# will-assistant/open-speech

Measured on AMD Instinct MI355X. Metric: audio-sec/sec (whisper-large-v3-turbo, 30 s clips, greedy), higher is better.
Workload: dtype f16; 1 GPU; large-v3-turbo: 64 x 30 s clips per GPU per step, mel+encoder+greedy decode (max_length 448); clips_per_gpu=64, global_batch=64, parallelism=dp1, lanes_per_gpu=3

## Files before the change

### include/osw.h

```cpp
#ifndef OSW_H
#define OSW_H

#include <stdint.h>

#ifdef __cplusplus
extern "C" {
#endif

#define OSW_OK 0
#define OSW_EINVAL (-22)
#define OSW_ENOMEM (-12)
#define OSW_EHIP (-100)
#define OSW_ESTATE (-101)
#define OSW_ECAPTURE (-102)

typedef struct osw_ctx osw_ctx;

typedef struct osw_dims {
    int32_t n_mels, n_audio_ctx, n_audio_state, n_audio_head, n_audio_layer;
    int32_t n_vocab, n_text_ctx, n_text_state, n_text_head, n_text_layer;
} osw_dims;

typedef struct osw_window {
    int32_t clip;
// ... 200 lines not shown

#define OSW_EPI_F16 0
#define OSW_EPI_F16_GELU 1
#define OSW_EPI_F32_RESID 2
#define OSW_EPI_F32_GELU_POS 3
#define OSW_EPI_F32 4
#define OSW_EPI_HEADS 5
typedef struct osw_enc_gemm_desc {
    int32_t M, N, K, variant, epi;
    int32_t heads_T, heads_H, heads_nb;
    int64_t lda, a_grp_rows, a_grp_stride;
    int64_t a_count;
    int64_t ldc, c_grp_rows, c_grp_stride, c_offset;
    int64_t c_bytes;
    int64_t pos_count;
    const void* A;
    const void* W;
    const float* bias;
    const float* pos;
    const int32_t* heads_slot;
    void* C;
} osw_enc_gemm_desc;
int osw_debug_enc_gemm(osw_ctx* ctx, const osw_enc_gemm_desc* desc);
int osw_debug_enc_layernorm(osw_ctx* ctx, int32_t M, int32_t M_alloc, int32_t D, const float* x, const float* gain,
                            const float* shift, void* y);

int osw_debug_get_logmel(osw_ctx* ctx, int32_t clip, float* out, int64_t out_floats, float* clip_max);
int osw_debug_mel_windows(osw_ctx* ctx, const osw_window* windows, int32_t n, void* out_halfs, int64_t out_count);

int osw_debug_hold_capture(osw_ctx* ctx, int32_t hold_ms);

int osw_set_profiling(osw_ctx* ctx, int32_t enable);
int osw_get_profile(osw_ctx* ctx, osw_profile* out);
void* osw_stream(osw_ctx* ctx);

int osw_ingest_mean_square(int32_t device, const int16_t* pcm, int64_t n_frames, int32_t channels, float* out_mean);
int osw_ingest_apply_gain(int32_t device, const int16_t* pcm, int64_t n_frames, int32_t channels, int32_t apply_gain,
                          float gain, int16_t* out);
int osw_ingest_resample(int32_t device, const int16_t* pcm, int64_t n_in, int32_t up, int32_t down, const float* h,
                        int32_t n_h, int16_t* out, int64_t n_out);

#ifdef __cplusplus
}
#endif
#endif
```

### open-speech_amd/_lib.py

```python
from __future__ import annotations

import ctypes as C
import os
import threading

_HERE = os.path.dirname(os.path.abspath(__file__))
LIB_PATH = os.environ.get("OSW_LIB", os.path.join(_HERE, "lib", "libosw_hip.so"))

OSW_OK = 0


class osw_dims(C.Structure):
    _fields_ = [(n, C.c_int32) for n in ("n_mels", "n_audio_ctx", "n_audio_state", "n_audio_head", "n_audio_layer",
                                          "n_vocab", "n_text_ctx", "n_text_state", "n_text_head", "n_text_layer")]


class osw_window(C.Structure):
    _fields_ = [("clip", C.c_int32), ("seek", C.c_int32), ("segment_size", C.c_int32)]


class osw_decode_opts(C.Structure):
    _fields_ = [("task_token", C.c_int32), ("language_token", C.c_int32), ("suppress_blank", C.c_int32),
                ("without_timestamps", C.c_int32), ("max_initial_timestamp_index", C.c_int32),
                ("max_length", C.c_int32), ("suppress_tokens", C.POINTER(C.c_int32)), ("n_suppress", C.c_int32),
# ... 118 lines not shown
                                      C.c_int32, C.c_int32, C.c_int32, P(C.c_float)]),
    "osw_debug_dec_xattn_windows": (C.c_int, [C.c_void_p, P(C.c_float), C.c_int32, P(C.c_float), C.c_void_p,
                                              C.c_void_p, C.c_int32, P(C.c_int32), C.c_int32, C.c_int32, C.c_int32,
                                              P(C.c_float)]),
    "osw_debug_dec_self_attn": (C.c_int, [C.c_void_p, P(C.c_float), C.c_int32, P(C.c_float), C.c_void_p, C.c_void_p,
                                          C.c_int32, P(C.c_int32), C.c_int32, P(C.c_int32), C.c_int32,
                                          P(C.c_float)]),
    "osw_debug_dec_gemm": (C.c_int, [C.c_void_p, C.c_int32, C.c_int32, C.c_int32, C.c_int32, C.c_void_p, C.c_void_p,
                                     C.c_void_p, C.c_int32, P(C.c_float), C.c_int64, P(C.c_int32)]),
    "osw_debug_dec_gemm_quant": (C.c_int, [C.c_void_p, C.c_int32, C.c_int32, C.c_int32, C.c_int32, C.c_void_p,
                                        C.c_void_p, C.c_void_p, P(C.c_float), C.c_int32, P(C.c_float), C.c_int64,
                                        P(C.c_int32)]),
    "osw_debug_dec_gemm_time": (C.c_int, [C.c_void_p, C.c_int32, C.c_int32, C.c_int32, C.c_void_p, C.c_void_p,
                                          C.c_void_p, P(C.c_float), C.c_int32, C.c_int32, C.c_int32, P(C.c_float),
                                          P(C.c_float)]),
    "osw_debug_logits_profile": (C.c_int, [C.c_void_p, P(C.c_double), P(C.c_int64)]),
    "osw_debug_dec_resln": (C.c_int, [C.c_void_p, C.c_int32, C.c_int32, C.c_int32, C.c_int32, P(C.c_float), C.c_int32,
                                      P(C.c_float), P(C.c_float), P(C.c_float), P(C.c_float), C.c_void_p,
                                      P(C.c_float), P(C.c_int32), P(C.c_int32), C.c_int32, C.c_int32, C.c_int32,
                                      C.c_void_p, C.c_int32, C.c_int32, P(C.c_float), C.c_void_p, C.c_void_p,
                                      P(C.c_float), C.c_int64, P(C.c_int32)]),
    "osw_debug_dec_gelu": (C.c_int, [C.c_void_p, C.c_int32, C.c_int32, C.c_int32, P(C.c_float), C.c_int32,
                                     P(C.c_float), C.c_void_p, C.c_int32, C.c_int32, C.c_void_p, C.c_void_p,
                                     P(C.c_float), C.c_int64, P(C.c_int32)]),
    "osw_debug_enc_gemm": (C.c_int, [C.c_void_p, P(osw_enc_gemm_desc)]),
    "osw_debug_enc_layernorm": (C.c_int, [C.c_void_p, C.c_int32, C.c_int32, C.c_int32, P(C.c_float), P(C.c_float),
                                          P(C.c_float), C.c_void_p]),
    "osw_debug_get_logmel": (C.c_int, [C.c_void_p, C.c_int32, P(C.c_float), C.c_int64, P(C.c_float)]),
    "osw_debug_mel_windows": (C.c_int, [C.c_void_p, P(osw_window), C.c_int32, C.c_void_p, C.c_int64]),
    "osw_debug_hold_capture": (C.c_int, [C.c_void_p, C.c_int32]),
    "osw_set_encoder_baton_min": (C.c_int, [C.c_void_p, C.c_int32]),
    "osw_set_profiling": (C.c_int, [C.c_void_p, C.c_int32]),
    "osw_get_profile": (C.c_int, [C.c_void_p, P(osw_profile)]),
    "osw_stream": (C.c_void_p, [C.c_void_p]),
    "osw_ingest_mean_square": (C.c_int, [C.c_int32, P(C.c_int16), C.c_int64, C.c_int32, P(C.c_float)]),
    "osw_ingest_apply_gain": (C.c_int, [C.c_int32, P(C.c_int16), C.c_int64, C.c_int32, C.c_int32, C.c_float,
                                        P(C.c_int16)]),
    "osw_ingest_resample": (C.c_int, [C.c_int32, P(C.c_int16), C.c_int64, C.c_int32, C.c_int32, P(C.c_float),
                                      C.c_int32, P(C.c_int16), C.c_int64]),
}
EXPORTED = tuple(_SIGS)

_lib = None
_lock = threading.Lock()


def load() -> C.CDLL:
    global _lib
    with _lock:
        if _lib is not None:
            return _lib
        if not os.path.exists(LIB_PATH):
            raise RuntimeError(f"libosw_hip.so not found at {LIB_PATH}: build it with `python __graft_entry__.py` "
                               "or `make -C open-speech_amd/csrc` (there is no CPU fallback)")
        lib = C.CDLL(LIB_PATH)
        for name, (res, args) in _SIGS.items():
            fn = getattr(lib, name)
            fn.restype = res
            fn.argtypes = args
        _lib = lib
        return lib


OSW_EINVAL = -22
OSW_EHIP = -100
OSW_ESTATE = -101
# ... 25 lines not shown
```

### open-speech_amd/csrc/common.h

```cpp
#pragma once
#include <hip/hip_runtime.h>
#include <hip/hip_fp16.h>
#include <stdint.h>

namespace osw {

typedef _Float16 h16;
typedef _Float16 h16x8 __attribute__((ext_vector_type(8)));
typedef _Float16 h16x4 __attribute__((ext_vector_type(4)));
typedef _Float16 h16x2 __attribute__((ext_vector_type(2)));
typedef float f32x4 __attribute__((ext_vector_type(4)));
typedef float f32x2 __attribute__((ext_vector_type(2)));
typedef float f32x16 __attribute__((ext_vector_type(16)));
typedef short s16x4 __attribute__((vector_size(8)));

#define OSW_LDS __attribute__((address_space(3)))

__device__ __forceinline__ int float_to_ordered(float f) {
    int i = __float_as_int(f);
    return i >= 0 ? i : (i ^ 0x7fffffff);
}
__device__ __forceinline__ float ordered_to_float(int i) {
    return __int_as_float(i >= 0 ? i : (i ^ 0x7fffffff));
}
// ... 64 lines not shown
    EPI_F32_GELU_POS = 3,
    EPI_F32 = 4,
    EPI_HEADS = 5,
};

struct GemmArgs {
    const h16* A; int64_t lda; int64_t a_grp_rows; int64_t a_grp_stride;
    const h16* W; int64_t ldw;
    const float* bias;
    int M, N, K;
    void* C; int64_t ldc; int64_t c_grp_rows; int64_t c_grp_stride;
    const float* pos;
    int epi;
    int heads_T, heads_H, heads_nb;
    const int* heads_slot;
    int band;
    int kc;
    const h16* A_lo;
    int preload_w;
    int pair_rows;
    int share_cus;
    const h16* Wf;
    const float* wscale;
    const int8_t* Wq;
};

__device__ __forceinline__ void split_h16(float v, h16* hi, h16* lo, int64_t i) {
    const h16 h = (h16)v;
    hi[i] = h;
    lo[i] = (h16)(v - (float)h);
}

void launch_gemm(const GemmArgs& g, hipStream_t s);
void launch_frag_pack(const h16* W, int64_t ldw, int N, int K, h16* Wf, hipStream_t s);
void launch_frag_pack_q8(const int8_t* q, int N, int K, int8_t* Wq, hipStream_t s);
void launch_gemm_variant(const GemmArgs& g, int variant, hipStream_t s);
void launch_gemm_skinny(const GemmArgs& g, float* part, hipStream_t s);
int skinny_ksplit(int N, int K);
void prepare_gemm_kernels();
int tiled_ksplit(int M, int N, int K);
void launch_gemm_tiled_partial(const GemmArgs& g, float* part, int ks, hipStream_t s);
int launch_gemm_skinny_partial(const GemmArgs& g, float* part, hipStream_t s);
struct ProArgs;
int launch_gemm_skinny_gelu_tail(const GemmArgs& g, float* part, const ProArgs& pa, hipStream_t s);
int launch_gemm_skinny_pro(const GemmArgs& g, int pro, const ProArgs& pa, bool direct, float* part, hipStream_t s,
                           bool select = false, bool attn_tail = false);
void launch_layernorm(const float* x, int64_t M, int D, const float* g, const float* b, h16* y, hipStream_t s);
bool layernorm_width_ok(int D);

}
```

### open-speech_amd/csrc/ctx.h

```cpp
#pragma once
#include <hip/hip_runtime.h>

#include <atomic>
#include <chrono>
#include <cmath>
#include <cstdio>
#include <cstdlib>
#include <cstring>
#include <deque>
#include <map>
#include <pthread.h>
#include <functional>
#include <memory>
#include <mutex>
#include <stdexcept>
#include <string>
#include <thread>
#include <vector>

#include "../../include/osw.h"
#include "common.h"
#include "align.h"
#include "decode.h"
#include "plan.h"
#include "resln.h"

namespace osw {
void launch_mel(const int16_t*, const int64_t*, const int64_t*, const int*, int, int, const float2*, const float*,
                const int*, const int*, const int*, const float*, int, float*, int*, hipStream_t);
void launch_mel_window(const float*, const int64_t*, const int*, const int*, const int*, const int*, const int*, int,
                       int, int, int, h16*, hipStream_t);
void launch_mel_normalize(const float*, int64_t, int, int, const int*, int, float*, hipStream_t);
void launch_enc_attn(const h16*, h16*, int, int, int, hipStream_t);
void launch_enc_attn_form(const h16*, h16*, int, int, int, bool eager, bool small, bool pipe, int grid_cap,
                          hipStream_t);
void launch_init_uniform(void*, bool, int64_t, uint64_t, float, float, int64_t, int64_t, hipStream_t);
uint64_t hash_stream_key(uint64_t, int64_t);
void launch_dec_self_attn(const float*, int, const float*, h16*, h16*, const int*, int, int, int, h16*, int64_t,
                          const int*, int, const SelState*, hipStream_t, int pos_row = 0);
void launch_dec_cross_attn(const float*, int, const float*, const h16*, const h16*, int, int, int, int, h16*, int64_t,
                           float*, int*, const SelState*, hipStream_t, const int* wmap = nullptr,
                           bool full = false);
void launch_dec_resid_ln(const float*, int, int, int, const float*, float*, const float*, const float*, h16*, int64_t,
                         const h16*, const float*, const int*, const int*, int, int, hipStream_t, int pos_row = 0,
                         const float* tok_scale = nullptr);
void launch_dec_reduce_gelu(const float*, int, int, int, const float*, h16*, int64_t, hipStream_t);
void launch_ingest_sumsq(const int16_t*, int, int, const int2*, int, float*, float*, hipStream_t);
void launch_ingest_gain(const int16_t*, int64_t, int, int, float, int16_t*, hipStream_t);
void launch_ingest_resample(const int16_t*, int64_t, const float*, int, int, int, int64_t, int64_t, int16_t*,
                            hipStream_t);

extern thread_local std::string g_err;

inline int hip_code(hipError_t e) {
    switch (e) {
        case hipErrorStreamCaptureUnsupported:
// ... 65 lines not shown
        if (*it == (void*)p) {
            owned.erase(it);
            break;
        }
    GateLock gate_(capture_gate());
    (void)hipFree(p);
    p = nullptr;
}

struct DeviceScope {
    int prev = -1;
    explicit DeviceScope(int device) {
        HIPCHK(hipGetDevice(&prev));
        if (prev != device) HIPCHK(hipSetDevice(device));
    }
    ~DeviceScope() {
        int cur = -1;
        if (prev >= 0 && hipGetDevice(&cur) == hipSuccess && cur != prev) (void)hipSetDevice(prev);
    }
    DeviceScope(const DeviceScope&) = delete;
    DeviceScope& operator=(const DeviceScope&) = delete;
};

struct EventPair {
    hipEvent_t a, b;
    int cls;
    double work;
};

struct EncBaton {
    std::mutex mu;
    hipEvent_t ev = nullptr;
    bool recorded = false;
    std::atomic<int> in_call{0};
    ~EncBaton() {
        if (ev) (void)hipEventDestroy(ev);
    }
};

struct AlignBufs {
    int *slot = nullptr, *len = nullptr, *forced = nullptr, *lh = nullptr;
    int *slot_len = nullptr, *slot_frames = nullptr, *slot_width = nullptr, *slot_T = nullptr, *path_len = nullptr;
    int *head = nullptr, *slot_head = nullptr;
    int *tf = nullptr, *path = nullptr;
    float *tokprob = nullptr , *scores = nullptr, *stats = nullptr, *colstats = nullptr, *M = nullptr;
    unsigned char* trace = nullptr;
    float *kc32 = nullptr, *vc32 = nullptr;
    int cap_slots = 0, cap_pstride = 0, cap_heads = 0, cap_rows = 0;
    int64_t gen = 0;
    std::vector<int> heads;
    std::vector<int> layer_first;
    int n_heads = 0;
    bool heads_dirty = true;
    std::vector<int> win, T, F;
    int pstride = 0;
};
}

using namespace osw;

struct osw_ctx {
    std::mutex mu;
    int device = 0;
    hipStream_t stream = nullptr;
    osw_dims d{};
    int B = 0;
    int R = 0;
    int C1 = 0;
    int T = 0;
    int NF = 0;
    std::vector<void*> owned;
    std::map<std::string, Tensor> w;
    std::shared_ptr<void> arena;
    std::shared_ptr<std::atomic<int>> siblings;
    bool sibling = false;
    bool finalized = false;
    std::shared_ptr<EncBaton> baton;
    int baton_min = 9;
    bool share_cus = false;
    hipStream_t enc_stream = nullptr;
    hipEvent_t enc_in = nullptr, enc_out = nullptr;

    float2* tw400 = nullptr;
    float* hann = nullptr;
    int *flo = nullptr, *fcnt = nullptr, *foff = nullptr;
    float* fw = nullptr;
    int16_t* pcm = nullptr;
    size_t pcm_cap = 0;
    int64_t* offsets = nullptr;
    int64_t* mel_off_d = nullptr;
    int* nframes_d = nullptr;
    int* clip_max = nullptr;
    int clips_cap = 0;
    float* logmel = nullptr;
    size_t logmel_cap = 0;
    int n_clips = 0;
    std::vector<int> nframes;
    std::vector<int64_t> mel_off;

    int* win = nullptr;
    h16 *X1 = nullptr, *H1 = nullptr, *Xn = nullptr, *QKV = nullptr, *O = nullptr, *Hf = nullptr, *E = nullptr,
        *XKV = nullptr;
    float* X = nullptr;
    int n_encoded = 0;
    bool row_pos = false;
    int kv_rows = 0;
    int xkv_windows = 0;
    struct Session* sess = nullptr;
    struct ClipStore* cstore = nullptr;
    int* slot_d = nullptr;
    int* refill_pack = nullptr;

// ... 49 lines not shown
    std::vector<EventPair> evs;
    std::vector<hipEvent_t> ev_free;
};

namespace osw {

void trace_graph(const osw_ctx* c, const char* what);
hipEvent_t get_ev(osw_ctx* c);

enum { CL_ENC_GEMM = 1, CL_ENC_ATTN = 2, CL_MEL = 3, CL_XATTN = 4, CL_LOGITS = 5, CL_STAGE_MEL = 10, CL_STAGE_ENC = 11,
       CL_STAGE_XKV = 12, CL_STAGE_DEC = 13 };

struct Timed {
    osw_ctx* c;
    EventPair p{};
    bool on;
    Timed(osw_ctx* c_, int cls, double work) : c(c_), on(c_->prof && !c_->capturing) {
        if (!on) return;
        p.a = get_ev(c);
        p.b = get_ev(c);
        p.cls = cls;
        p.work = work;
        HIPCHK(hipEventRecord(p.a, c->stream));
    }
    ~Timed() {
        if (!on) return;
        if (hipEventRecord(p.b, c->stream) == hipSuccess) c->evs.push_back(p);
    }
};

struct LaneCall {
    osw_ctx* c;
    explicit LaneCall(osw_ctx* c_) : c(c_) {
        c->share_cus = c->baton && c->baton->in_call.fetch_add(1) > 0;
    }
    ~LaneCall() {
        if (c->baton) c->baton->in_call.fetch_sub(1);
    }
};

void resolve_events(osw_ctx* c);
Tensor& W(osw_ctx* c, const std::string& n);
const h16* WH(osw_ctx* c, const std::string& n);
const float* WF(osw_ctx* c, const std::string& n);
const h16* WFR(osw_ctx* c, const std::string& n);
bool is_q8(osw_ctx* c, const std::string& n);
void gemm_weights(osw_ctx* c, const std::string& n, GemmArgs& g);
void require_embedding_kind(osw_ctx* c);
const float* tok_scale(osw_ctx* c);
GemmArgs gemm_plain(const h16* A, int64_t lda, const h16* Wt, const float* bias, int M, int N, int K, void* C,
                    int64_t ldc, int epi);
bool skinny_ok(const GemmArgs& g);
void run_gemm(osw_ctx* c, const GemmArgs& g0, int cls);
void encoder_layer(osw_ctx* c, int i, int nb);
std::vector<int> pack_windows(osw_ctx* c, const osw_window* wins, int n);
void encode(osw_ctx* c, const osw_window* wins, int n, const int* slots = nullptr);
void reserve_clips(osw_ctx* c, int n);

bool decoder_step(osw_ctx* c, int nb, int group, bool gather, const SelFuse* sf = nullptr);
hipGraphExec_t decode_graph(osw_ctx* c, const std::vector<int64_t>& key, const std::function<void()>& one_step,
                            int CH);
void decode(osw_ctx* c, int nb, const osw_decode_opts* o, osw_window_result* r, const int32_t* windows = nullptr);
void detect_language(osw_ctx* c, int nb, const osw_decode_opts* o, float* probs, float* raw);
void decode_refill(osw_ctx* c, int n_clips, const osw_decode_opts* o, osw_window_result* r, int refill_min);
struct Readback {
    std::vector<SelState> st;
    std::vector<BeamWin> bw;
    std::vector<int> toks;
    std::vector<float> cum, lang;
};
// ... 13 lines not shown
```

### open-speech_amd/csrc/gemm.hip

```cpp
#include "common.h"
#include "resln.h"

#include <cstdlib>
#include <mutex>
#include <set>
#include <stdexcept>

namespace osw {

namespace {
#include "select.h"
constexpr int HD = 64;
#include "selfattn.h"

constexpr int BM = 128, BN = 128, BK = 64, NTHR = 256;
#ifndef OSW_SKINNY_CK1
#define OSW_SKINNY_CK1 4
#endif

void set_lds_once(const void* kernel, int bytes) {
    static std::mutex mu;
    static std::set<const void*> done;
    std::lock_guard<std::mutex> lk(mu);
    if (done.insert(kernel).second) (void)hipFuncSetAttribute(kernel, hipFuncAttributeMaxDynamicSharedMemorySize, bytes);
}

__device__ __forceinline__ int heads_window(const GemmArgs& g, int b) { return g.heads_slot ? g.heads_slot[b] : b; }

__device__ __forceinline__ int swz(int row, int chunk) { return chunk ^ ((row >> 1) & 7); }

__device__ __forceinline__ int fast_div(int m, int d) {
    if (m >= (1 << 22)) return m / d;
    int q = (int)((float)m * __builtin_amdgcn_rcpf((float)d));
    const int r = m - q * d;
    q += (r >= d ? 1 : 0) - (r < 0 ? 1 : 0);
    return q;
}

__device__ __forceinline__ int64_t c_row(const GemmArgs& g, int m) {
    if (g.c_grp_rows >= g.M) return (int64_t)m * g.ldc;
    const int q = fast_div(m, g.c_grp_rows);
// ... 843 lines not shown
}

template <int EPI, int DBG = 0>
__global__ __launch_bounds__(GNT, 1) void gemm8p_kernel(GemmArgs g) {
    extern __shared__ __attribute__((aligned(16))) h16 smem[];
    const int nwg = ((g.N + GB - 1) / GB) * ((g.M + GB - 1) / GB);
    const bool next0 = g.kc == 1 && (g.K / BK) % 2 == 0;
    bool pre0 = false;
    for (int vb = blockIdx.x; vb < nwg; vb += gridDim.x) {
        int tid = threadIdx.x;
        asm volatile("" : "+v"(tid));
        const int nxt = next0 && vb + (int)gridDim.x < nwg ? vb + (int)gridDim.x : -1;
        gemm8p_tile<EPI, DBG>(g, vb, smem, tid, pre0, nxt);
        pre0 = nxt >= 0;
        if (!pre0) __syncthreads();
    }
}

int grid8(const GemmArgs& g) {
    static const int cus = [] {
        int dev = 0, n = 0;
        if (hipGetDevice(&dev) != hipSuccess || hipDeviceGetAttribute(&n, hipDeviceAttributeMultiprocessorCount, dev) != hipSuccess)
            return 256;
        return n;
    }();
    static const bool per_tile = [] {
        const char* e = std::getenv("OSW_GEMM_PERSIST");
        return e && e[0] == '0';
    }();
    static const int shared_cap = [] {
        if (const char* gg = std::getenv("OSW_GEMM_GRID")) return std::max(8, std::min(cus, atoi(gg)) / 8 * 8);
        return std::max(8, cus * 3 / 4 / 8 * 8);
    }();
    return per_tile ? 1 << 30 : std::max(8, g.share_cus ? shared_cap : cus);
}

template <int EPI, int DBG = 0>
void launch8p(const GemmArgs& g0, hipStream_t s) {
    constexpr int lds = EPI_LDS > 8 * HT * 2 ? EPI_LDS : 8 * HT * 2;
    set_lds_once((const void*)gemm8p_kernel<EPI, DBG>, lds);
    GemmArgs g = g0;
    g.band = choose_band(g);
    static const int next0_env = [] {
        const char* e = std::getenv("OSW_GEMM_NEXT0");
        return e ? (e[0] == '1' ? 1 : 0) : -1;
    }();
    const bool next0 = next0_env < 0 ? EPI == EPI_F16_GELU : next0_env == 1;
    g.kc = next0 ? 1 : 0;
    const int nwg = ((g.N + GB - 1) / GB) * ((g.M + GB - 1) / GB);
    gemm8p_kernel<EPI, DBG><<<std::min(nwg, grid8(g)), GNT, lds, s>>>(g);
}

constexpr int H8_SLOTS = 3, H8_LDS = H8_SLOTS * 3 * HT * 2;
static_assert(H8_LDS >= EPI_LDS, "the epilogue image fits the ring");

template <int EPI, int DBG>
__device__ __forceinline__ void gemm8h_tile(const GemmArgs& g, int bid, h16* smem, int tid) {
    const int wave = tid >> 6, lane = tid & 63;
    constexpr bool TR = EPI == EPI_F16 || EPI == EPI_F16_GELU;
    int m0, n0;
    tile8p_origin<128>(g, bid, m0, n0);
    const h16* src[3][2];
#pragma unroll
    for (int H = 0; H < 3; ++H)
#pragma unroll
        for (int i = 0; i < 2; ++i) src[H][i] = src8p(g, m0, n0, H, i, wave, lane);
    auto stage = [&](int H, int t) {
        h16* base = smem + ((t % H8_SLOTS) * 3 + H) * HT;
#pragma unroll
        for (int i = 0; i < 2; ++i)
            __builtin_amdgcn_global_load_lds((const void*)(src[H][i] + t * BK),
                                             (OSW_LDS void*)(base + (i * 8 + wave) * 8 * BK), 16, 0, 0);
    };
    const int wm = wave >> 2, wn = wave & 3;
    const int li = lane & 15, lc = lane >> 4;
    const int aoff0 = (wm * 64 + li) * BK + swz(wm * 64 + li, lc) * 8;
    const int aoff1 = (wm * 64 + li) * BK + swz(wm * 64 + li, 4 + lc) * 8;
    const int boff0 = (wn * 32 + li) * BK + swz(wn * 32 + li, lc) * 8;
    const int boff1 = (wn * 32 + li) * BK + swz(wn * 32 + li, 4 + lc) * 8;
    f32x4 acc[8][4];
#pragma unroll
    for (int i = 0; i < 8; ++i)
// ... 91 lines not shown
        staged_epilogue<EPI, true, TR, 128>(g, acc, m0, n0, wm, wn, (char*)smem, tid);
    }
}

template <int EPI, int DBG = 0>
__global__ __launch_bounds__(GNT, 1) void gemm8h_kernel(GemmArgs g) {
    extern __shared__ __attribute__((aligned(16))) h16 smem[];
    const int nwg = ((g.N + 127) / 128) * ((g.M + GB - 1) / GB);
    for (int vb = blockIdx.x; vb < nwg; vb += gridDim.x) {
        int tid = threadIdx.x;
        asm volatile("" : "+v"(tid));
        gemm8h_tile<EPI, DBG>(g, vb, smem, tid);
        __syncthreads();
    }
}

bool use_half_tile(const GemmArgs& g, int64_t t8) {
    static const bool on = [] {
        const char* e = std::getenv("OSW_GEMM_HALF");
        return !(e && e[0] == '0');
    }();
    if (!on || g.A_lo || g.kc != 0 || g.N % 8 != 0 || t8 < 90 || t8 >= 512) return false;
    if (t8 < 180 && g.epi != EPI_F32_RESID && g.epi != EPI_F32) return false;
    const int64_t G = grid8(g), th = (int64_t)((g.N + 127) / 128) * ((g.M + GB - 1) / GB);
    return ((th + G - 1) / G) < 2 * ((t8 + G - 1) / G);
}

template <int EPI, int DBG = 0>
void launch8h(const GemmArgs& g0, hipStream_t s) {
    set_lds_once((const void*)gemm8h_kernel<EPI, DBG>, H8_LDS);
    GemmArgs g = g0;
    g.band = choose_band(g, 128);
    const int nwg = ((g.N + 127) / 128) * ((g.M + GB - 1) / GB);
    gemm8h_kernel<EPI, DBG><<<std::min(nwg, grid8(g)), GNT, H8_LDS, s>>>(g);
}


template <int N>
__device__ __forceinline__ void wait_vmcnt() {
    static_assert(N < 64, "vmcnt range");
    __builtin_amdgcn_s_waitcnt((N & 15) | ((N >> 4) << 14) | (7 << 4) | (15 << 8));
}

constexpr int R128_NS = 4, R128_SLOT = 2 * 128 * BK;
constexpr int R128_LDS = R128_NS * R128_SLOT * 2;

template <int EPI>
__global__ __launch_bounds__(NTHR, 1) void gemm128_ring_kernel(GemmArgs g) {
    constexpr int TM = 128, PW = 4, FT = 4, WT = 64;
    extern __shared__ __attribute__((aligned(16))) h16 smem[];
    const int wave = threadIdx.x >> 6, lane = threadIdx.x & 63;
    const int ntm = (g.M + TM - 1) / TM, ntn = (g.N + TM - 1) / TM, nwg = ntm * ntn;
    const int bid = blockIdx.x, q = nwg / 8, r8 = nwg % 8, xcd = bid % 8;
    const int v = (xcd < r8 ? xcd * (q + 1) : r8 * (q + 1) + (xcd - r8) * q) + bid / 8;
    const int m0 = (v % ntm) * TM, n0 = (v / ntm) * TM;
    const h16* asrc[PW];
    const h16* wsrc[PW];
#pragma unroll
    for (int i = 0; i < PW; ++i) {
        const int r = (i * 4 + wave) * 8 + (lane >> 3);
        const int c = swz(r, lane & 7);
        asrc[i] = grp_row(g.A, min(m0 + r, g.M - 1), g.a_grp_rows, g.a_grp_stride, g.lda) + c * 8;
        wsrc[i] = g.W + (int64_t)min(n0 + r, g.N - 1) * g.ldw + c * 8;
    }
    auto stage = [&](int slot, int k0) {
        h16* base = smem + slot * R128_SLOT;
// ... 1229 lines not shown
```

### open-speech_amd/csrc/osw.hip

```cpp
#include "ctx.h"

namespace osw {
thread_local std::string g_err;

std::recursive_mutex& capture_gate() {
    static std::recursive_mutex m;
    return m;
}

void trace_graph(const osw_ctx* c, const char* what) {
    static const bool on = [] {
        const char* e = std::getenv("OSW_TRACE_GRAPH");
        return e && e[0] == '1';
    }();
    if (!on) return;
    std::fprintf(stderr, "[osw-graph] thread %zx ctx %p %s\n", (size_t)pthread_self(), (const void*)c, what);
    std::fflush(stderr);
}

hipEvent_t get_ev(osw_ctx* c) {
    if (!c->ev_free.empty()) {
        hipEvent_t e = c->ev_free.back();
        c->ev_free.pop_back();
        return e;
// ... 316 lines not shown
    GateLock gate_(capture_gate());
    HIPCHK(hipHostMalloc((void**)&c->done_host, sizeof(int), 0));
}

GemmArgs gemm_plain(const h16* A, int64_t lda, const h16* Wt, const float* bias, int M, int N, int K, void* C,
                    int64_t ldc, int epi) {
    GemmArgs g{};
    g.A = A; g.lda = lda; g.a_grp_rows = M; g.a_grp_stride = 0;
    g.W = Wt; g.ldw = K; g.bias = bias; g.M = M; g.N = N; g.K = K;
    g.C = C; g.ldc = ldc; g.c_grp_rows = M; g.c_grp_stride = 0; g.pos = nullptr; g.epi = epi;
    return g;
}

bool skinny_ok(const GemmArgs& g) {
    if (g.N >= 16384 && g.M >= 24) return false;
    return g.M <= 64 && g.K % 128 == 0 &&
           (g.epi == EPI_F16 || g.epi == EPI_F16_GELU || g.epi == EPI_F32_RESID || g.epi == EPI_F32);
}

void run_gemm(osw_ctx* c, const GemmArgs& g0, int cls) {
    GemmArgs g = g0;
    g.share_cus = c->share_cus;
    REQUIRE(g.K % 64 == 0, "GEMM K must be a multiple of 64");
    REQUIRE(!g.A_lo || g.epi == EPI_F32, "hi/lo operands feed fp32 outputs only");
    const bool skinny = skinny_ok(g);
    REQUIRE(skinny || g.epi == EPI_F32 ||
                (g.N % 8 == 0 && (g.epi == EPI_HEADS || (g.ldc % 8 == 0 && g.c_grp_stride % 8 == 0))),
            "GEMM epilogue needs N, ldc and the C group stride to be multiples of 8");
    Timed t(c, cls, 2.0 * g.M * g.N * g.K);
    if (skinny) {
        REQUIRE((int64_t)skinny_ksplit(g.N, g.K) * g.M * g.N <= c->part_floats, "split-K workspace too small");
        launch_gemm_skinny(g, c->part, c->stream);
    } else {
        launch_gemm(g, c->stream);
    }
    HIPCHK(hipGetLastError());
}

void encoder_layer(osw_ctx* c, int i, int nb) {
    const osw_dims& d = c->d;
    const int De = d.n_audio_state, H = d.n_audio_head;
    const int M = nb * c->T;
    const std::string p = "enc.l" + std::to_string(i);
    launch_layernorm(c->X, M, De, WF(c, p + ".ln1.g"), WF(c, p + ".ln1.b"), c->Xn, c->stream);
    GemmArgs g = gemm_plain(c->Xn, De, WH(c, p + ".qkv.w"), WF(c, p + ".qkv.b"), M, 3 * De, De, c->QKV, 0, EPI_HEADS);
    g.heads_T = c->T; g.heads_H = H; g.heads_nb = nb;
    run_gemm(c, g, CL_ENC_GEMM);
    {
        Timed t(c, CL_ENC_ATTN, 4.0 * nb * H * (double)c->T * c->T * 64);
        launch_enc_attn(c->QKV, c->O, c->T, H, nb, c->stream);
        HIPCHK(hipGetLastError());
    }
    run_gemm(c, gemm_plain(c->O, De, WH(c, p + ".o.w"), WF(c, p + ".o.b"), M, De, De, c->X, De, EPI_F32_RESID),
             CL_ENC_GEMM);
    launch_layernorm(c->X, M, De, WF(c, p + ".ln2.g"), WF(c, p + ".ln2.b"), c->Xn, c->stream);
    run_gemm(c, gemm_plain(c->Xn, De, WH(c, p + ".fc1.w"), WF(c, p + ".fc1.b"), M, 4 * De, De, c->Hf, 4 * De,
                           EPI_F16_GELU), CL_ENC_GEMM);
    run_gemm(c, gemm_plain(c->Hf, 4 * De, WH(c, p + ".fc2.w"), WF(c, p + ".fc2.b"), M, De, 4 * De, c->X, De,
                           EPI_F32_RESID), CL_ENC_GEMM);
}

std::vector<int> pack_windows(osw_ctx* c, const osw_window* wins, int n) {
    std::vector<int> hw(3 * (size_t)n);
    for (int i = 0; i < n; ++i) {
        REQUIRE(wins[i].clip >= 0 && wins[i].clip < c->n_clips, "window clip out of range");
        REQUIRE(wins[i].seek >= 0 && wins[i].seek < c->nframes[wins[i].clip], "window seek out of range");
        REQUIRE(wins[i].segment_size >= 1, "empty window");
        hw[i] = wins[i].clip;
        hw[n + i] = wins[i].seek;
        hw[2 * n + i] = std::min(wins[i].segment_size, c->NF);
    }
    return hw;
}

void encode(osw_ctx* c, const osw_window* wins, int n, const int* slots) {
    REQUIRE(c->finalized, "weights not finalized");
    REQUIRE(n >= 1 && n <= c->B, "window count out of range");
    const osw_dims& d = c->d;
    const int De = d.n_audio_state;
    if (slots) {
        std::vector<char> seen(c->B, 0);
        for (int i = 0; i < n; ++i) {
            REQUIRE(slots[i] >= 0 && slots[i] < c->B && !seen[slots[i]], "refill slots must be distinct rows < max_batch");
            seen[slots[i]] = 1;
        }
    }
    const std::vector<int> hw = pack_windows(c, wins, n);
    HIPCHK(hipMemcpyAsync(c->win, hw.data(), hw.size() * 4, hipMemcpyHostToDevice, c->stream));
    std::unique_lock<std::mutex> baton;
    if (c->baton && n >= c->baton_min) baton = std::unique_lock<std::mutex>(c->baton->mu);
    hipStream_t dec_stream = c->stream;
    struct Restore {
        osw_ctx* c;
        hipStream_t s;
        bool share;
        ~Restore() { c->stream = s; c->share_cus = share; }
    } restore{c, dec_stream, c->share_cus};
    static const bool share_small = getenv("OSW_SHARE_SMALL") != nullptr;
    if (n < c->baton_min && !share_small) c->share_cus = false;
    if (c->enc_stream) {
        HIPCHK(hipEventRecord(c->enc_in, dec_stream));
        HIPCHK(hipStreamWaitEvent(c->enc_stream, c->enc_in, 0));
        c->stream = c->enc_stream;
    }
    if (baton.owns_lock() && c->baton->recorded) HIPCHK(hipStreamWaitEvent(c->stream, c->baton->ev, 0));
    {
        Timed t(c, CL_STAGE_ENC, 0);
        launch_mel_window(c->logmel, c->mel_off_d, c->nframes_d, c->clip_max, c->win, c->win + n, c->win + 2 * n, n,
                          d.n_mels, c->C1, c->NF, c->X1, c->stream);
        GemmArgs g{};
        g.A = c->X1; g.lda = c->C1; g.a_grp_rows = c->NF; g.a_grp_stride = (c->NF + 2LL) * c->C1;
        g.W = WH(c, "enc.conv1.w"); g.ldw = 3 * c->C1; g.bias = WF(c, "enc.conv1.b");
        g.M = n * c->NF; g.N = De; g.K = 3 * c->C1;
        g.C = c->H1 + De; g.ldc = De; g.c_grp_rows = c->NF; g.c_grp_stride = (c->NF + 1LL) * De; g.epi = EPI_F16_GELU;
        run_gemm(c, g, CL_ENC_GEMM);
        GemmArgs g2{};
        g2.A = c->H1; g2.lda = 2LL * De; g2.a_grp_rows = c->T; g2.a_grp_stride = (c->NF + 1LL) * De;
        g2.W = WH(c, "enc.conv2.w"); g2.ldw = 3LL * De; g2.bias = WF(c, "enc.conv2.b");
        g2.M = n * c->T; g2.N = De; g2.K = 3 * De;
        g2.C = c->X; g2.ldc = De; g2.c_grp_rows = c->T; g2.c_grp_stride = (int64_t)c->T * De;
        g2.pos = WF(c, "enc.pos"); g2.epi = EPI_F32_GELU_POS;
        run_gemm(c, g2, CL_ENC_GEMM);
        for (int i = 0; i < d.n_audio_layer; ++i) encoder_layer(c, i, n);
        launch_layernorm(c->X, (int64_t)n * c->T, De, WF(c, "enc.lnpost.g"), WF(c, "enc.lnpost.b"), c->E, c->stream);
    }
    {
        Timed t(c, CL_STAGE_XKV, 0);
        GemmArgs g = gemm_plain(c->E, De, WH(c, "dec.crosskv.w"), WF(c, "dec.crosskv.b"), n * c->T,
                                d.n_text_layer * 2 * d.n_text_state, De, c->XKV, 0, EPI_HEADS);
        g.heads_T = c->T; g.heads_H = d.n_text_head; g.heads_nb = n;
        if (slots) {
            HIPCHK(hipMemcpyAsync(c->slot_d, slots, (size_t)n * 4, hipMemcpyHostToDevice, c->stream));
            g.heads_nb = c->B;
            g.heads_slot = c->slot_d;
        }
        run_gemm(c, g, 0);
    }
    HIPCHK(hipGetLastError());
    if (baton.owns_lock()) {
        HIPCHK(hipEventRecord(c->baton->ev, c->stream));
        c->baton->recorded = true;
    }
    if (c->enc_stream) {
        HIPCHK(hipEventRecord(c->enc_out, c->enc_stream));
        HIPCHK(hipStreamWaitEvent(dec_stream, c->enc_out, 0));
    }
    c->n_encoded = n;
}

void align_sync_heads(osw_ctx* c) {
    AlignBufs& A = c->al;
    const int L = c->d.n_text_layer, H = c->d.n_text_head;
    if (!A.heads_dirty) return;
    std::vector<int> hd = A.heads;
    if (hd.empty())
        for (int l = L - L / 2; l < L; ++l)
            for (int h = 0; h < H; ++h) {
                hd.push_back(l);
                hd.push_back(h);
            }
    const int n = (int)hd.size() / 2;
    if (!A.lh) A.lh = dalloc<int>((size_t)2 * L * H, c->owned);
    std::vector<int> lh;
    A.layer_first.assign(L + 1, 0);
    for (int l = 0; l < L; ++l) {
        A.layer_first[l] = (int)lh.size() / 2;
        for (int i = 0; i < n; ++i)
            if (hd[2 * i] == l) {
                lh.push_back(hd[2 * i + 1]);
                lh.push_back(i);
            }
    }
    A.layer_first[L] = (int)lh.size() / 2;
    HIPCHK(hipMemcpyAsync(A.lh, lh.data(), lh.size() * 4, hipMemcpyHostToDevice, c->stream));
    HIPCHK(hipStreamSynchronize(c->stream));
    A.n_heads = n;
    A.heads_dirty = false;
    ++A.gen;
}

// ... 343 lines not shown
        f();
        resolve_events(c);
    });
}
}

extern "C" {

const char* osw_version(void) { return "osw-hip 0.2 gfx950"; }
const char* osw_last_error(void) { return g_err.c_str(); }

int osw_device_count(int32_t* out) {
    return guard([&] {
        int n = 0;
        HIPCHK(hipGetDeviceCount(&n));
        *out = n;
    });
}

void make_streams(osw_ctx* c) {
    const char* ep = std::getenv("OSW_ENC_PRIO");
    if (!ep || ep[0] != '1') {
        HIPCHK(hipStreamCreateWithFlags(&c->stream, hipStreamNonBlocking));
        return;
    }
    int lo = 0, hi = 0;
    HIPCHK(hipDeviceGetStreamPriorityRange(&lo, &hi));
    HIPCHK(hipStreamCreateWithPriority(&c->stream, hipStreamNonBlocking, hi));
    HIPCHK(hipStreamCreateWithPriority(&c->enc_stream, hipStreamNonBlocking, lo));
    HIPCHK(hipEventCreateWithFlags(&c->enc_in, hipEventDisableTiming));
    HIPCHK(hipEventCreateWithFlags(&c->enc_out, hipEventDisableTiming));
}

void destroy_streams(osw_ctx* c) {
    if (c->stream) (void)hipStreamDestroy(c->stream);
    if (c->enc_stream) (void)hipStreamDestroy(c->enc_stream);
    if (c->enc_in) (void)hipEventDestroy(c->enc_in);
    if (c->enc_out) (void)hipEventDestroy(c->enc_out);
}

static int drop_partial(osw_ctx* c, int rc) {
    if (!c) return rc;
    GateLock gate_(capture_gate());
    for (void* p : c->owned) (void)hipFree(p);
    destroy_streams(c);
    delete c;
    return rc;
}

int osw_create(const osw_dims* dims, int32_t device, int32_t max_batch, osw_ctx** out) {
    osw_ctx* c = nullptr;
    int rc = guard([&] {
        REQUIRE(dims && out, "null argument");
        REQUIRE(max_batch >= 1 && max_batch <= 1024, "max_batch out of range");
        REQUIRE(dims->n_audio_state % 128 == 0 && dims->n_text_state % 128 == 0, "model width must be a multiple of 128");
        REQUIRE(dims->n_audio_state / dims->n_audio_head == 64 && dims->n_text_state / dims->n_text_head == 64,
                "head_dim must be 64");
        REQUIRE(dims->n_audio_ctx >= 50 && dims->n_audio_ctx <= 1500 && dims->n_audio_ctx % 50 == 0,
                "n_audio_ctx must be 50 * chunk_length, chunk_length 1..30 (50, 100, ..., 1500)");
        REQUIRE((XCHUNKS - 1) * ((dims->n_audio_ctx + XCHUNKS - 1) / XCHUNKS) < dims->n_audio_ctx,
                "n_audio_ctx leaves a cross-attention key chunk empty");
        REQUIRE(dims->n_text_ctx <= 448, "n_text_ctx must be <= 448");
        REQUIRE(dims->n_audio_state == dims->n_text_state, "encoder and decoder width must match");
        REQUIRE(dims->n_audio_state <= 1280, "model width > 1280 unsupported");
        REQUIRE(layernorm_width_ok(dims->n_audio_state),
                "model width must be one of 128, 256, 384, 512, 768, 1024, 1280 (no LayerNorm kernel for 640, 896, 1152)");
        int ndev = 0;
        HIPCHK(hipGetDeviceCount(&ndev));
        REQUIRE(device >= 0 && device < ndev, "device ordinal out of range");
        GateLock gate_(capture_gate());
        c = new osw_ctx();
        c->device = device;
        c->d = *dims;
        c->B = max_batch;
        c->R = max_batch * 5;
        c->C1 = (dims->n_mels + 63) / 64 * 64;
        c->T = dims->n_audio_ctx;
        c->NF = 2 * c->T;
        if (const char* e = std::getenv("OSW_NO_GRAPH")) c->use_graph = !(e[0] == '1');
        if (const char* e = std::getenv("OSW_BATON_MIN_WINDOWS")) c->baton_min = atoi(e);
        DeviceScope dev_scope_((device));
        prepare_gemm_kernels();
        make_streams(c);
        const char* eb = std::getenv("OSW_ENC_BATON");
        if (!eb || eb[0] != '0') {
            c->baton = std::make_shared<EncBaton>();
            HIPCHK(hipEventCreateWithFlags(&c->baton->ev, hipEventDisableTiming));
        }
        build_weight_table(c);
        setup_mel(c);
        setup_workspace(c);
        HIPCHK(hipStreamSynchronize(c->stream));
        *out = c;
    });
    return rc == OSW_OK ? rc : drop_partial(c, rc);
}

int osw_create_sibling(osw_ctx* parent, int32_t max_batch, osw_ctx** out) {
    osw_ctx* c = nullptr;
    int rc = guard([&] {
        REQUIRE(parent && out, "null argument");
        REQUIRE(max_batch >= 1 && max_batch <= 1024, "max_batch out of range");
        std::lock_guard<std::mutex> lk(parent->mu);
        REQUIRE(parent->finalized, "parent context weights not finalized");
        GateLock gate_(capture_gate());
        c = new osw_ctx();
        c->device = parent->device;
        c->d = parent->d;
        c->B = max_batch;
        c->R = max_batch * 5;
        c->C1 = parent->C1;
        c->T = parent->T;
        c->NF = parent->NF;
        c->use_graph = parent->use_graph;
        c->baton_min = parent->baton_min;
        DeviceScope dev_scope_((c->device));
        make_streams(c);
        c->w = parent->w;
        c->arena = parent->arena;
        c->siblings = parent->siblings;
        if (c->siblings) c->siblings->fetch_add(1);
        c->baton = parent->baton;
        c->sibling = true;
        c->finalized = true;
        setup_mel(c);
        setup_workspace(c);
        HIPCHK(hipStreamSynchronize(c->stream));
        *out = c;
    });
    return rc == OSW_OK ? rc : drop_partial(c, rc);
}

int osw_destroy(osw_ctx* c) {
    if (!c) return OSW_OK;
    return guard([&] {
        {
            std::lock_guard<std::mutex> lk(c->mu);
            DeviceScope dev_scope_((c->device));
            HIPCHK(hipStreamSynchronize(c->stream));
            GateLock gate_(capture_gate());
            for (auto& e : c->evs) { (void)hipEventDestroy(e.a); (void)hipEventDestroy(e.b); }
            for (auto e : c->ev_free) (void)hipEventDestroy(e);
            for (auto& kv : c->dgraphs) (void)hipGraphExecDestroy(kv.second.first);
            session_destroy(c);
            for (void* p : c->owned) (void)hipFree(p);
            if (c->done_host) (void)hipHostFree(c->done_host);
            destroy_streams(c);
            if (c->sibling && c->siblings) c->siblings->fetch_sub(1);
            c->arena.reset();
        }
// ... 284 lines not shown
            wins[i] = osw_window{i, 0, std::max(1, std::min(c->NF, c->nframes[i] - 1))};
        encode(c, wins.data(), n_clips);
        decode(c, n_clips, opts, res);
    });
}

int osw_transcribe_refill(osw_ctx* c, const int16_t* pcm, const int64_t* offsets, int32_t n_clips,
                          int32_t pcm_on_device, const osw_decode_opts* opts, osw_window_result* res,
                          int32_t refill_min) {
    return lane_call(c, c, "null ctx", [&] {
        REQUIRE(n_clips >= 1, "n_clips out of range");
        log_mel(c, pcm, offsets, n_clips, pcm_on_device, nullptr);
        decode_refill(c, n_clips, opts, res, refill_min);
    });
}

int osw_set_encoder_baton_min(osw_ctx* c, int32_t min_windows) {
    return guard([&] {
        REQUIRE(c, "null ctx");
        REQUIRE(min_windows >= 0, "min_windows must be >= 0");
        std::lock_guard<std::mutex> lk(c->mu);
        c->baton_min = min_windows;
    });
}

int osw_set_profiling(osw_ctx* c, int32_t enable) {
    return guard([&] {
        REQUIRE(c, "null ctx");
        std::lock_guard<std::mutex> lk(c->mu);
        REQUIRE(enable >= 0 && enable <= 2, "profiling mode must be 0, 1 or 2");
        c->prof = enable != 0;
        c->prof_eager = enable == 2;
        c->pf = osw_profile{};
        c->logits_ms = 0;
        c->logits_launches = 0;
    });
}

int osw_get_profile(osw_ctx* c, osw_profile* out) {
    return guard([&] {
        REQUIRE(c && out, "null argument");
        std::lock_guard<std::mutex> lk(c->mu);
        resolve_events(c);
        *out = c->pf;
    });
}

void* osw_stream(osw_ctx* c) { return c ? (void*)c->stream : nullptr; }

int osw_ingest_mean_square(int32_t device, const int16_t* pcm, int64_t n_frames, int32_t channels, float* out_mean) {
    return guard([&] {
        REQUIRE(pcm && out_mean, "null argument");
        REQUIRE(n_frames >= 1 && channels >= 1 && channels <= 64, "bad PCM shape");
        IngestDev& g = ingest_dev(device);
        std::lock_guard<std::mutex> lk(g.mu);
        DeviceScope dev_scope_((device));
        const size_t n = (size_t)n_frames * channels;
        grow(g.in, g.in_cap, n, g.owned);
        HIPCHK(hipMemcpyAsync(g.in, pcm, n * 2, hipMemcpyHostToDevice, g.s));
        *out_mean = ingest_mean_square(g, g.in, n_frames, channels);
    });
}

int osw_ingest_apply_gain(int32_t device, const int16_t* pcm, int64_t n_frames, int32_t channels, int32_t apply_gain,
                          float gain, int16_t* out) {
    return guard([&] {
        REQUIRE(pcm && out, "null argument");
        REQUIRE(n_frames >= 1 && channels >= 1 && channels <= 64, "bad PCM shape");
        IngestDev& g = ingest_dev(device);
        std::lock_guard<std::mutex> lk(g.mu);
        DeviceScope dev_scope_((device));
        const size_t n = (size_t)n_frames * channels;
        grow(g.in, g.in_cap, n, g.owned);
        grow(g.out, g.out_cap, (size_t)n_frames, g.owned);
        HIPCHK(hipMemcpyAsync(g.in, pcm, n * 2, hipMemcpyHostToDevice, g.s));
        launch_ingest_gain(g.in, n_frames, channels, apply_gain, gain, g.out, g.s);
        HIPCHK(hipGetLastError());
// ... 41 lines not shown
```

### open-speech_amd/engine.py

```python
from __future__ import annotations

import ctypes as C
import dataclasses
from dataclasses import dataclass, field

import numpy as np

from . import _lib
from .dims import SpecialTokens, WhisperDims
from .weights import F16, canonical_specs, make_tensor


@dataclass
class DecodeConfig:
    task: str = "transcribe"
    language_token: int | None = None
    suppress_tokens: tuple = ()
    suppress_blank: bool = True
    without_timestamps: bool = False
    max_initial_timestamp_index: int | None = 50
    max_length: int = 448
    beam_size: int = 1
    patience: float = 1.0
    length_penalty: float = 1.0
# ... 787 lines not shown
        fp = C.POINTER(C.c_float)
        _lib.check(self.lib.osw_debug_enc_layernorm(self.ctx, M, out.shape[0], Dm, x.ctypes.data_as(fp),
                                                    g.ctypes.data_as(fp), b.ctypes.data_as(fp),
                                                    out.ctypes.data_as(C.c_void_p)), "osw_debug_enc_layernorm")
        return out

    def debug_get_logmel(self, clip: int) -> tuple[np.ndarray, np.float32]:
        out = np.empty((self._nframes[clip], self.dims.n_mels), np.float32)
        mx = C.c_float()
        _lib.check(self.lib.osw_debug_get_logmel(self.ctx, int(clip), out.ctypes.data_as(C.POINTER(C.c_float)),
                                                 out.size, C.byref(mx)), "osw_debug_get_logmel")
        return out, np.float32(mx.value)

    def debug_mel_windows(self, windows: list) -> np.ndarray:
        arr = (_lib.osw_window * len(windows))(*[_lib.osw_window(int(c), int(s), int(z)) for c, s, z in windows])
        c1 = (self.dims.n_mels + 63) // 64 * 64
        out = np.empty((len(windows), 2 * self.dims.n_audio_ctx + 2, c1), np.float16)
        _lib.check(self.lib.osw_debug_mel_windows(self.ctx, arr, len(windows), out.ctypes.data_as(C.c_void_p),
                                                  out.size), "osw_debug_mel_windows")
        return out

    def hold_capture(self, hold_ms: int) -> None:
        _lib.check(self.lib.osw_debug_hold_capture(self.ctx, int(hold_ms)), "osw_debug_hold_capture")

    def set_encoder_baton_min(self, min_windows: int) -> None:
        _lib.check(self.lib.osw_set_encoder_baton_min(self.ctx, int(min_windows)), "osw_set_encoder_baton_min")

    def set_profiling(self, on: bool, eager_decode: bool = False) -> None:
        _lib.check(self.lib.osw_set_profiling(self.ctx, 2 if on and eager_decode else int(on)), "osw_set_profiling")

    def profile(self) -> dict:
        p = _lib.osw_profile()
        _lib.check(self.lib.osw_get_profile(self.ctx, C.byref(p)), "osw_get_profile")
        return p.as_dict()

    def stream(self) -> int:
        return int(self.lib.osw_stream(self.ctx) or 0)

    def close(self) -> None:
        if getattr(self, "ctx", None):
            self.lib.osw_destroy(self.ctx)
            self.ctx = None

    def __del__(self):
        try:
            self.close()
        except Exception:
            pass
```

Before: 5226 audio-sec/sec.

## Share CUs with sibling lanes during encoder via due-count and layer pacing

```diff
diff --git a/include/osw.h b/include/osw.h
--- a/include/osw.h
+++ b/include/osw.h
@@ -256,6 +256,7 @@
 
 int osw_set_profiling(osw_ctx* ctx, int32_t enable);
 int osw_get_profile(osw_ctx* ctx, osw_profile* out);
+int osw_get_grid_counts(osw_ctx* ctx, int64_t* full_grid, int64_t* shared_grid, int64_t* encoders);
 void* osw_stream(osw_ctx* ctx);
 
 int osw_ingest_mean_square(int32_t device, const int16_t* pcm, int64_t n_frames, int32_t channels, float* out_mean);
diff --git a/open-speech_amd/_lib.py b/open-speech_amd/_lib.py
--- a/open-speech_amd/_lib.py
+++ b/open-speech_amd/_lib.py
@@ -174,6 +174,7 @@
     "osw_set_encoder_baton_min": (C.c_int, [C.c_void_p, C.c_int32]),
     "osw_set_profiling": (C.c_int, [C.c_void_p, C.c_int32]),
     "osw_get_profile": (C.c_int, [C.c_void_p, P(osw_profile)]),
+    "osw_get_grid_counts": (C.c_int, [C.c_void_p, P(C.c_int64), P(C.c_int64), P(C.c_int64)]),
     "osw_stream": (C.c_void_p, [C.c_void_p]),
     "osw_ingest_mean_square": (C.c_int, [C.c_int32, P(C.c_int16), C.c_int64, C.c_int32, P(C.c_float)]),
     "osw_ingest_apply_gain": (C.c_int, [C.c_int32, P(C.c_int16), C.c_int64, C.c_int32, C.c_int32, C.c_float,
diff --git a/open-speech_amd/csrc/common.h b/open-speech_amd/csrc/common.h
--- a/open-speech_amd/csrc/common.h
+++ b/open-speech_amd/csrc/common.h
@@ -120,6 +120,7 @@
 }
 
 void launch_gemm(const GemmArgs& g, hipStream_t s);
+extern thread_local int g_grid8_launches;
 void launch_frag_pack(const h16* W, int64_t ldw, int N, int K, h16* Wf, hipStream_t s);
 void launch_frag_pack_q8(const int8_t* q, int N, int K, int8_t* Wq, hipStream_t s);
 void launch_gemm_variant(const GemmArgs& g, int variant, hipStream_t s);
diff --git a/open-speech_amd/csrc/ctx.h b/open-speech_amd/csrc/ctx.h
--- a/open-speech_amd/csrc/ctx.h
+++ b/open-speech_amd/csrc/ctx.h
@@ -22,6 +22,7 @@
 #include "common.h"
 #include "align.h"
 #include "decode.h"
+#include "encshare.h"
 #include "plan.h"
 #include "resln.h"
 
@@ -153,7 +154,7 @@
     std::mutex mu;
     hipEvent_t ev = nullptr;
     bool recorded = false;
-    std::atomic<int> in_call{0};
+    EncShare share;
     ~EncBaton() {
         if (ev) (void)hipEventDestroy(ev);
     }
@@ -198,7 +199,11 @@
     bool finalized = false;
     std::shared_ptr<EncBaton> baton;
     int baton_min = 9;
-    bool share_cus = false;
+    int share_cus = 0;
+    EncShareLane lane;
+    hipEvent_t pace_ev[EncPacer::RING] = {};
+    std::atomic<int64_t> grid_full{0}, grid_shared{0};
+    std::atomic<int64_t> enc_enqueued{0};
     hipStream_t enc_stream = nullptr;
     hipEvent_t enc_in = nullptr, enc_out = nullptr;
 
@@ -314,10 +319,11 @@
 struct LaneCall {
     osw_ctx* c;
     explicit LaneCall(osw_ctx* c_) : c(c_) {
-        c->share_cus = c->baton && c->baton->in_call.fetch_add(1) > 0;
+        c->share_cus = 0;
+        if (c->baton) c->lane.begin_call(c->baton->share);
     }
     ~LaneCall() {
-        if (c->baton) c->baton->in_call.fetch_sub(1);
+        if (c->baton) c->lane.end_call(c->baton->share);
     }
 };
 
diff --git a/open-speech_amd/csrc/encshare.h b/open-speech_amd/csrc/encshare.h
--- /dev/null
+++ b/open-speech_amd/csrc/encshare.h
@@ -0,0 +1,65 @@
+#pragma once
+#include <algorithm>
+#include <atomic>
+#include <cstdlib>
+
+namespace osw {
+
+struct EncShare {
+    std::atomic<int> due{0};
+    std::atomic<int> in_call{0};
+};
+
+struct EncShareLane {
+    bool counted = false;
+    bool call_share = false;
+    void begin_call(EncShare& s) {
+        counted = false;
+        call_share = s.in_call.fetch_add(1) > 0;
+    }
+    void take_baton(EncShare& s) {
+        if (counted) return;
+        counted = true;
+        s.due.fetch_add(1);
+    }
+    void end_call(EncShare& s) {
+        s.in_call.fetch_sub(1);
+        if (counted) s.due.fetch_sub(1);
+        counted = false;
+        call_share = false;
+    }
+    int siblings_due(const EncShare& s) const { return std::max(0, s.due.load() - (counted ? 1 : 0)); }
+    int decide(const EncShare& s, bool holds_baton, bool per_call) const {
+        if (!holds_baton) return 0;
+        return per_call ? (call_share ? 2 : 0) : siblings_due(s);
+    }
+};
+
+struct EncPacer {
+    static constexpr int RING = 8;
+    int lookahead = 2;
+    explicit EncPacer(int la = 2) : lookahead(std::min(RING, std::max(0, la))) {}
+    bool on() const { return lookahead > 0; }
+    static int slot(int layer) { return layer % RING; }
+    int wait_layer(int layer, bool share) const {
+        return share && lookahead > 0 && layer >= lookahead ? layer - lookahead : -1;
+    }
+};
+
+inline bool enc_share_per_call() {
+    static const bool v = [] {
+        const char* e = std::getenv("OSW_ENC_SHARE");
+        return e && e[0] == 'c';
+    }();
+    return v;
+}
+
+inline int enc_lookahead() {
+    static const int v = [] {
+        const char* e = std::getenv("OSW_ENC_LOOKAHEAD");
+        return e ? std::atoi(e) : 2;
+    }();
+    return v;
+}
+
+}
diff --git a/open-speech_amd/csrc/gemm.hip b/open-speech_amd/csrc/gemm.hip
--- a/open-speech_amd/csrc/gemm.hip
+++ b/open-speech_amd/csrc/gemm.hip
@@ -7,6 +7,8 @@
 #include <stdexcept>
 
 namespace osw {
+
+thread_local int g_grid8_launches = 0;
 
 namespace {
 #include "select.h"
@@ -916,7 +918,7 @@
         if (const char* gg = std::getenv("OSW_GEMM_GRID")) return std::max(8, std::min(cus, atoi(gg)) / 8 * 8);
         return std::max(8, cus * 3 / 4 / 8 * 8);
     }();
-    return per_tile ? 1 << 30 : std::max(8, g.share_cus ? shared_cap : cus);
+    return per_tile ? 1 << 30 : std::max(8, g.share_cus > 0 ? shared_cap : cus);
 }
 
 template <int EPI, int DBG = 0>
@@ -932,6 +934,7 @@
     const bool next0 = next0_env < 0 ? EPI == EPI_F16_GELU : next0_env == 1;
     g.kc = next0 ? 1 : 0;
     const int nwg = ((g.N + GB - 1) / GB) * ((g.M + GB - 1) / GB);
+    ++g_grid8_launches;
     gemm8p_kernel<EPI, DBG><<<std::min(nwg, grid8(g)), GNT, lds, s>>>(g);
 }
 
@@ -1089,6 +1092,7 @@
     GemmArgs g = g0;
     g.band = choose_band(g, 128);
     const int nwg = ((g.N + 127) / 128) * ((g.M + GB - 1) / GB);
+    ++g_grid8_launches;
     gemm8h_kernel<EPI, DBG><<<std::min(nwg, grid8(g)), GNT, H8_LDS, s>>>(g);
 }
 
diff --git a/open-speech_amd/csrc/osw.hip b/open-speech_amd/csrc/osw.hip
--- a/open-speech_amd/csrc/osw.hip
+++ b/open-speech_amd/csrc/osw.hip
@@ -372,7 +372,9 @@
         REQUIRE((int64_t)skinny_ksplit(g.N, g.K) * g.M * g.N <= c->part_floats, "split-K workspace too small");
         launch_gemm_skinny(g, c->part, c->stream);
     } else {
+        const int before = g_grid8_launches;
         launch_gemm(g, c->stream);
+        if (g_grid8_launches != before && !c->capturing) ++(g.share_cus ? c->grid_shared : c->grid_full);
     }
     HIPCHK(hipGetLastError());
 }
@@ -433,11 +435,25 @@
     struct Restore {
         osw_ctx* c;
         hipStream_t s;
-        bool share;
-        ~Restore() { c->stream = s; c->share_cus = share; }
-    } restore{c, dec_stream, c->share_cus};
+        ~Restore() { c->stream = s; c->share_cus = 0; }
+    } restore{c, dec_stream};
     static const bool share_small = getenv("OSW_SHARE_SMALL") != nullptr;
-    if (n < c->baton_min && !share_small) c->share_cus = false;
+    const bool holds = baton.owns_lock();
+    const bool per_call = enc_share_per_call() || !holds;
+    if (holds) c->lane.take_baton(c->baton->share);
+    auto decide = [&] {
+        c->share_cus = c->baton ? c->lane.decide(c->baton->share, holds || share_small, per_call) : 0;
+    };
+    const EncPacer pacer(holds && !per_call && !c->capturing && !c->prof_eager ? enc_lookahead() : 0);
+    auto pace = [&](int layer) {
+        decide();
+        const int w = pacer.wait_layer(layer, c->share_cus > 0);
+        if (w >= 0) HIPCHK(hipEventSynchronize(c->pace_ev[EncPacer::slot(w)]));
+    };
+    auto paced = [&](int layer) {
+        if (pacer.on()) HIPCHK(hipEventRecord(c->pace_ev[EncPacer::slot(layer)], c->stream));
+    };
+    decide();
     if (c->enc_stream) {
         HIPCHK(hipEventRecord(c->enc_in, dec_stream));
         HIPCHK(hipStreamWaitEvent(c->enc_stream, c->enc_in, 0));
@@ -461,9 +477,14 @@
         g2.C = c->X; g2.ldc = De; g2.c_grp_rows = c->T; g2.c_grp_stride = (int64_t)c->T * De;
         g2.pos = WF(c, "enc.pos"); g2.epi = EPI_F32_GELU_POS;
         run_gemm(c, g2, CL_ENC_GEMM);
-        for (int i = 0; i < d.n_audio_layer; ++i) encoder_layer(c, i, n);
+        for (int i = 0; i < d.n_audio_layer; ++i) {
+            pace(i);
+            encoder_layer(c, i, n);
+            paced(i);
+        }
         launch_layernorm(c->X, (int64_t)n * c->T, De, WF(c, "enc.lnpost.g"), WF(c, "enc.lnpost.b"), c->E, c->stream);
     }
+    pace(d.n_audio_layer);
     {
         Timed t(c, CL_STAGE_XKV, 0);
         GemmArgs g = gemm_plain(c->E, De, WH(c, "dec.crosskv.w"), WF(c, "dec.crosskv.b"), n * c->T,
@@ -486,6 +507,7 @@
         HIPCHK(hipStreamWaitEvent(dec_stream, c->enc_out, 0));
     }
     c->n_encoded = n;
+    ++c->enc_enqueued;
 }
 
 void align_sync_heads(osw_ctx* c) {
@@ -895,11 +917,17 @@
     HIPCHK(hipEventCreateWithFlags(&c->enc_out, hipEventDisableTiming));
 }
 
+void make_pace_events(osw_ctx* c) {
+    for (hipEvent_t& e : c->pace_ev) HIPCHK(hipEventCreateWithFlags(&e, hipEventDisableTiming));
+}
+
 void destroy_streams(osw_ctx* c) {
     if (c->stream) (void)hipStreamDestroy(c->stream);
     if (c->enc_stream) (void)hipStreamDestroy(c->enc_stream);
     if (c->enc_in) (void)hipEventDestroy(c->enc_in);
     if (c->enc_out) (void)hipEventDestroy(c->enc_out);
+    for (hipEvent_t e : c->pace_ev)
+        if (e) (void)hipEventDestroy(e);
 }
 
 static int drop_partial(osw_ctx* c, int rc) {
@@ -945,6 +973,7 @@
         DeviceScope dev_scope_((device));
         prepare_gemm_kernels();
         make_streams(c);
+        make_pace_events(c);
         const char* eb = std::getenv("OSW_ENC_BATON");
         if (!eb || eb[0] != '0') {
             c->baton = std::make_shared<EncBaton>();
@@ -979,6 +1008,7 @@
         c->baton_min = parent->baton_min;
         DeviceScope dev_scope_((c->device));
         make_streams(c);
+        make_pace_events(c);
         c->w = parent->w;
         c->arena = parent->arena;
         c->siblings = parent->siblings;
@@ -1329,6 +1359,9 @@
         c->prof = enable != 0;
         c->prof_eager = enable == 2;
         c->pf = osw_profile{};
+        c->grid_full = 0;
+        c->grid_shared = 0;
+        c->enc_enqueued = 0;
         c->logits_ms = 0;
         c->logits_launches = 0;
     });
@@ -1340,6 +1373,15 @@
         std::lock_guard<std::mutex> lk(c->mu);
         resolve_events(c);
         *out = c->pf;
+    });
+}
+
+int osw_get_grid_counts(osw_ctx* c, int64_t* full_grid, int64_t* shared_grid, int64_t* encoders) {
+    return guard([&] {
+        REQUIRE(c && full_grid && shared_grid && encoders, "null argument");
+        *encoders = c->enc_enqueued.load();
+        *full_grid = c->grid_full.load();
+        *shared_grid = c->grid_shared.load();
     });
 }
 
diff --git a/open-speech_amd/engine.py b/open-speech_amd/engine.py
--- a/open-speech_amd/engine.py
+++ b/open-speech_amd/engine.py
@@ -843,7 +843,15 @@
     def profile(self) -> dict:
         p = _lib.osw_profile()
         _lib.check(self.lib.osw_get_profile(self.ctx, C.byref(p)), "osw_get_profile")
-        return p.as_dict()
+        out = p.as_dict()
+        out["enc_gemm_full_grid"], out["enc_gemm_shared_grid"], _ = self.grid_counts()
+        return out
+
+    def grid_counts(self) -> tuple:
+        full, shared, enc = C.c_int64(0), C.c_int64(0), C.c_int64(0)
+        _lib.check(self.lib.osw_get_grid_counts(self.ctx, C.byref(full), C.byref(shared), C.byref(enc)),
+                   "osw_get_grid_counts")
+        return full.value, shared.value, enc.value
 
     def stream(self) -> int:
         return int(self.lib.osw_stream(self.ctx) or 0)
```

After: 5227 audio-sec/sec (median of 3 runs). About the same (+0.0%).
